# lchdl/DeepWMH

Hardware: NVIDIA B200
Metric: volumes/sec (higher is better)
Workload: dtype f16

## Files before the change

### deepwmh_b200/csrc/conv_tcgen05.cuh

```cuda
#pragma once
#include <cuda.h>
#include <algorithm>
#include <cstdio>
#include <cstdlib>
#include <string>
#include <type_traits>
#include <vector>
#include "common.cuh"
#include "tc_primitives.cuh"

namespace dwmh {

constexpr int TC_WARPS_PER_GROUP = 7;
constexpr int TC_THREADS = 224;
constexpr int TC_TH = 16, TC_TW = 8;
constexpr int TC_PH = 18, TC_PW = 10;
constexpr int TC_PLANE_BYTES = TC_PH * TC_PW * 16;
constexpr int TC_MAX_SA = 4, TC_MAX_NB = 40, TC_MAX_R = 16;
constexpr int TC_SMEM_MAX = 232448;
constexpr int TC_SMEM_RESERVED = 5120;
constexpr int TC_SMEM_RESERVED_FIRST = 10240;
constexpr int TC_FIRST_PITCH = 12;
constexpr int TC_FIRST_SLICE = TC_PH * TC_FIRST_PITCH;
constexpr int TC_FIRST_STAGE_BYTES = 8 * 128 * 16;

struct TcClassDesc { int tapmask, jlo, jcnt, tile0; };

struct TcKParams {
  const void* wpack; void* out; StatPartial* partials;
  int C0, C1, Cout, CB, KC, nkc, nkc0;
  int nclass, Jlo, Jhi, jmax, tiles_per_kc, Din;
  int out32;
  int s222;
  int tconv, CBt, osd, osh, osw, Cout_t;
  TcClassDesc cls[8];
  int D, H, W, tilesH, tilesW, ZB, nzb, ncb;
  int SA, NB, resident, R, fmt;
  const double* xf_sums; const float* xf_gamma; const float* xf_beta; double xf_inv_count; int xform; const void* xf_src;
  const float* fc_src; const SampleMeta* fc_metas; int fc_patch_mode, fc_SY, fc_SZ, first;
  int stagger;
  int G;
  int total_items;
  unsigned long long* prof;
  int dbg;
  uint32_t a_stage_bytes, b_tile_bytes, off_b, off_bar;
};

__global__ void __launch_bounds__(256) stats_reduce_kernel(const StatPartial* __restrict__ partials, double* __restrict__ out,
                                                           int ncb, int CB, int Cout, int ipb, int jn) {
  __shared__ double sh[3][256];
  const int n = blockIdx.x / ncb, cb = blockIdx.x % ncb;
  const int c = threadIdx.x % CB, j = threadIdx.x / CB;
  const StatPartial* base = partials + (size_t)blockIdx.x * ipb * CB + c;
  double cn = 0.0, cm = 0.0, cq = 0.0;
  for (int p = j; p < ipb; p += jn) {
    const float4 v = *reinterpret_cast<const float4*>(base + (size_t)p * CB);
    stat_merge<double>(cn, cm, cq, (double)v.x, (double)v.y, (double)v.z);
  }
  sh[0][threadIdx.x] = cn; sh[1][threadIdx.x] = cm; sh[2][threadIdx.x] = cq;
  __syncthreads();
  if (j == 0) {
    for (int jj = 1; jj < jn; ++jj) stat_merge<double>(cn, cm, cq, sh[0][jj * CB + c], sh[1][jj * CB + c], sh[2][jj * CB + c]);
    double* o = out + ((size_t)n * Cout + (size_t)cb * CB + c) * 2;
    o[0] = cm;
    o[1] = cn > 0.0 ? cq / cn : 0.0;
  }
}

struct RingPos {
  uint32_t idx = 0, phase = 0;
  __device__ __forceinline__ void advance(uint32_t n) { if (++idx == n) { idx = 0; phase ^= 1; } }
  __device__ __forceinline__ RingPos next(uint32_t n) const { RingPos r = *this; r.advance(n); return r; }
};

#define DWMH_TIMED_WAIT(acc, ...) do { if (prof_on) { const long long t__ = clock64(); __VA_ARGS__; acc += clock64() - t__; } else { __VA_ARGS__; } } while (0)

__device__ __forceinline__ uint64_t tc_desc(uint32_t hi, uint32_t lo) { return ((uint64_t)hi << 32) | lo; }

constexpr uint64_t tc_tap_shift_table() {
  uint64_t v = 0;
  for (int sft = 0; sft < 9; ++sft) v |= (uint64_t)((sft / 3) * TC_PW + (sft % 3)) << (5 * sft);
  return v;
}
constexpr uint64_t kTapShift = tc_tap_shift_table();

template <typename T, int KSTEPS, bool SMALL_CB, bool TCONV, bool DUAL, bool XFORM, bool FIRST = false>
__global__ void __launch_bounds__((DUAL ? 2 : 1) * (TC_THREADS + ((FIRST || XFORM) ? 32 : 0)), 1)
conv3_tc_kernel(const __grid_constant__ CUtensorMap tmA0, const __grid_constant__ CUtensorMap tmA1, const TcKParams p) {
  extern __shared__ __align__(1024) uint8_t smem[];
  const uint32_t smem_base = tc::smem_u32(smem);
  const int warp_abs = threadIdx.x >> 5, lane = threadIdx.x & 31;
  constexpr int WPG = TC_WARPS_PER_GROUP;
  constexpr int TPG = WPG * 32;
  constexpr int NG = DUAL ? 2 : 1;
  constexpr bool EXTRA = FIRST || XFORM;
  int g, warp;
  if constexpr (!DUAL) {
    constexpr unsigned char kRole7[7] = {2, 3, 4, 5, 0, 6, 1};
    constexpr unsigned char kRole8[8] = {2, 3, 4, 5, 0, 6, 7, 1};
    g = 0; warp = EXTRA ? kRole8[warp_abs] : kRole7[warp_abs];
  } else if constexpr (!EXTRA) {
    constexpr unsigned char kGroup14[14] = {0, 0, 0, 0, 1, 1, 1, 1, 0, 1, 0, 1, 1, 0};
    constexpr unsigned char kRole14[14] = {2, 3, 4, 5, 2, 3, 4, 5, 0, 0, 6, 6, 1, 1};
    g = kGroup14[warp_abs]; warp = kRole14[warp_abs];
  } else {
    constexpr unsigned char kGroup16[16] = {0, 0, 0, 0, 1, 1, 1, 1, 0, 1, 1, 1, 0, 0, 1, 0};
    constexpr unsigned char kRole16[16] = {2, 3, 4, 5, 2, 3, 4, 5, 0, 0, 6, 7, 6, 7, 1, 1};
    g = kGroup16[warp_abs]; warp = kRole16[warp_abs];
  }
  const bool extra = warp == 7;

  int wi = blockIdx.x * p.G + g;
  const bool idle = wi >= p.total_items;
  if (idle) wi = p.total_items - 1;
  const int tw = wi % p.tilesW; wi /= p.tilesW;
  const int th = wi % p.tilesH; wi /= p.tilesH;
  const int zb = wi % p.nzb; wi /= p.nzb;
  const int cb = wi % p.ncb; wi /= p.ncb;
  const int n = wi;
  const int h0 = th * TC_TH, w0 = tw * TC_TW;
  const int z_lo = zb * p.ZB, z_end = min(p.D, z_lo + p.ZB);
  const uint32_t SA = p.SA, NB = p.NB, R = p.R, CB = p.CB;

  const uint32_t nbar = 3 * SA + 2 * NB + 2 * R;
  const uint32_t bar0 = smem_base + p.off_bar, bar = bar0 + (uint32_t)g * nbar * 8u;
  const uint32_t a_full = bar, a_empty = bar + 8u * SA;
  const uint32_t b_full = bar0 + 16u * SA, b_empty = b_full + 8u * NB;
  const uint32_t acc_full = bar + 16u * SA + 16u * NB, acc_empty = acc_full + 8u * R;
  const uint32_t a_ready = acc_empty + 8u * R;
  const uint32_t a_mma = (XFORM || FIRST) ? a_ready : a_full;
  uint32_t* tmem_ptr_smem = reinterpret_cast<uint32_t*>(smem + p.off_bar + 8 * nbar * p.G);
  const uint32_t aux_off = (p.off_bar + 8u * nbar * (uint32_t)p.G + 16u + 8u) & ~15u;
  float* s_coef = reinterpret_cast<float*>(smem + aux_off) + (size_t)p.G * 2 * CB + (size_t)g * 2 * 64;
  float* s_slice = reinterpret_cast<float*>(smem + aux_off) + (size_t)p.G * 2 * CB + (size_t)p.G * 2 * 64 + (size_t)g * 4 * TC_FIRST_SLICE;
  const uint32_t smem_a = smem_base + (uint32_t)g * SA * p.a_stage_bytes;
  const uint32_t smem_a_d = smem_a & 0x3FFFFu, smem_b_d = (smem_base + p.off_b) & 0x3FFFFu;
  const uint32_t s_full = smem_base + p.off_bar + TC_SMEM_RESERVED_FIRST - 128 + (uint32_t)g * 64u, s_empty = s_full + 32u;

  if (threadIdx.x == 0) {
    if constexpr (!FIRST) {
      tc::prefetch_tensormap(&tmA0);
      tc::prefetch_tensormap(&tmA1);
    }
    for (int gg = 0; gg < p.G; ++gg) {
      const uint32_t bg = bar0 + (uint32_t)gg * nbar * 8u;
      for (uint32_t s_ = 0; s_ < SA; ++s_) { tc::mbar_init(bg + 8 * s_, 1); tc::mbar_init(bg + 8 * (SA + s_), 1); }
      for (uint32_t s_ = 0; s_ < R; ++s_) { tc::mbar_init(bg + 16 * SA + 16 * NB + 8 * s_, 1); tc::mbar_init(bg + 16 * SA + 16 * NB + 8 * (R + s_), 4); }
      for (uint32_t s_ = 0; s_ < SA; ++s_) tc::mbar_init(bg + 16 * SA + 16 * NB + 16 * R + 8 * s_, XFORM ? 3 : 2);
    }
    if constexpr (FIRST)
      for (int gg = 0; gg < p.G; ++gg)
        for (uint32_t s_ = 0; s_ < 4; ++s_) {
          tc::mbar_init(smem_base + p.off_bar + TC_SMEM_RESERVED_FIRST - 128 + gg * 64 + 8 * s_, 1);
          tc::mbar_init(smem_base + p.off_bar + TC_SMEM_RESERVED_FIRST - 128 + gg * 64 + 32 + 8 * s_, 2);
        }
    const uint32_t nactive = (uint32_t)min(p.G, p.total_items - (int)blockIdx.x * p.G);
    for (uint32_t s_ = 0; s_ < NB; ++s_) { tc::mbar_init(b_full + 8 * s_, 1); tc::mbar_init(b_empty + 8 * s_, nactive); }
    tc::fence_barrier_init();
  }
  if (warp_abs == 1) tc::tmem_alloc(tc::smem_u32(tmem_ptr_smem), 512);
  if constexpr (XFORM) {
    for (int i = threadIdx.x; i < p.G * p.C0; i += blockDim.x) {
      const int gg = i / p.C0, c_ = i - gg * p.C0;
      const int item = min((int)blockIdx.x * p.G + gg, p.total_items - 1);
      const int n_gg = item / (p.tilesW * p.tilesH * p.nzb * p.ncb);
      NormParams np{p.xf_sums, p.xf_gamma, p.xf_beta, p.xf_inv_count};
      float a_, b_;
      norm_coeffs(np, n_gg, p.C0, c_, a_, b_);
      float* co = reinterpret_cast<float*>(smem + aux_off) + (size_t)p.G * 2 * CB + (size_t)gg * 2 * 64;
      co[c_] = a_; co[64 + c_] = b_;
    }
  }
  tc::tc_fence_before();
  __syncthreads();
  tc::tc_fence_after();
  const uint32_t tmem = *tmem_ptr_smem + (uint32_t)g * 256u;
  const bool prof_on = (p.dbg & 8) != 0;
  long long w0_ = 0, w1_ = 0, w2_ = 0, w3_ = 0;
  const long long tstart_ = clock64();

  if (idle) {
  } else
  if (FIRST && warp == 7) {
    int ox = 0, oy = 0, oz = 0, flip = 0;
    const float* src = p.fc_src;
    int SY = p.fc_SY, SZ = p.fc_SZ;
    if (p.fc_patch_mode) { src += (size_t)n * p.D * p.H * p.W; SY = p.H; SZ = p.W; }
    else { const SampleMeta m_ = p.fc_metas[n]; ox = m_.ox; oy = m_.oy; oz = m_.oz; flip = m_.flip; }
    int sgoff[6]; bool sin_[6];
#pragma unroll
    for (int i = 0; i < 6; ++i) {
      const int pos = lane + 32 * i;
      const int r = pos / TC_PW, c = pos - r * TC_PW;
// ... 188 lines not shown
            const int c8 = first ? (n * p.nclass + c) * (p.C0 >> 3) + kc * (2 * KSTEPS) : n * (p.C1 >> 3) + (kc - p.nkc0) * (2 * KSTEPS);
            tc::tma_load_4d(smem_a + a.idx * p.a_stage_bytes, first ? &tmA0 : &tmA1, a_full + 8 * a.idx, (w0 - 1) * 8, h0 - 1, t, c8);
          }
          a.advance(SA);
        }
      }
    }
  } else if (warp == 6) {
    const bool leader = tc::elect_one();
    const int ntile = p.nkc * p.tiles_per_kc;
    const uint8_t* wsrc = reinterpret_cast<const uint8_t*>(p.wpack) + (size_t)cb * ntile * p.b_tile_bytes;
    if (p.resident) {
      if (leader && g == 0)
        for (int t = 0; t < ntile; ++t) {
          tc::mbar_arrive_expect_tx(b_full + 8 * t, p.b_tile_bytes);
          tc::bulk_load(smem_base + p.off_b + t * p.b_tile_bytes, wsrc + (size_t)t * p.b_tile_bytes, p.b_tile_bytes, b_full + 8 * t);
        }
    } else if (g == 0) {
      RingPos b;
      for (int t = z_lo - p.Jhi; t <= z_end - 1 - p.Jlo; ++t) {
        if (t < 0 || t >= p.Din) continue;
        for (int c = 0; c < p.nclass; ++c) {
          if (max(t + p.cls[c].jlo, z_lo) > min(t + p.cls[c].jlo + p.cls[c].jcnt - 1, z_end - 1)) continue;
          const int ntaps = __popc(p.cls[c].tapmask);
          for (int kc = 0; kc < p.nkc; ++kc)
            for (int ti = 0; ti < ntaps; ++ti) {
              const int tile = kc * p.tiles_per_kc + p.cls[c].tile0 + ti;
              DWMH_TIMED_WAIT(w0_, tc::mbar_wait(b_empty + 8 * b.idx, b.phase ^ 1, 2));
              if (leader) {
                tc::mbar_arrive_expect_tx(b_full + 8 * b.idx, p.b_tile_bytes);
                tc::bulk_load(smem_base + p.off_b + b.idx * p.b_tile_bytes, wsrc + (size_t)tile * p.b_tile_bytes, p.b_tile_bytes, b_full + 8 * b.idx);
              }
              b.advance(NB);
            }
        }
      }
    }
  } else if (warp == 1) {
    const bool elected = tc::elect_one();
    const bool leader = elected && !(p.dbg & 2);
    if constexpr (FIRST) {
      const uint32_t idesc = tc::instr_desc_f16(p.fmt, 128, (int)CB);
      const uint32_t hi_desc = (128u >> 4) | (1u << 14);
      const uint32_t a_lbo = (2048u >> 4) << 16, b_lbo = ((CB * 16u) >> 4) << 16;
      const uint32_t b_lo0 = (smem_b_d >> 4) | b_lbo;
      tc::mbar_wait(b_full, 0, 5);
      RingPos a, fresh, done;
      for (int t = z_lo; t < z_end; ++t) {
        tc::mbar_wait(acc_empty + 8 * fresh.idx, fresh.phase ^ 1, 3);
        tc::mbar_wait(a_mma + 8 * a.idx, a.phase, 4);
        tc::tc_fence_after();
        if (leader) {
          const uint32_t a_lo0 = ((smem_a_d + a.idx * p.a_stage_bytes) >> 4) | a_lbo;
          const uint32_t col = tmem + fresh.idx * CB;
#pragma unroll
          for (int i = 0; i < 6; ++i) {
            const int achunk = (i == 0 || i == 4) ? 0 : (i == 1 || i == 5) ? 2 : (i == 2 ? 4 : 6);
            tc::umma_f16(col, tc_desc(hi_desc, a_lo0 + achunk * (2048 >> 4)), tc_desc(hi_desc, b_lo0 + i * 2 * CB), idesc, i == 0 ? 0u : 1u);
          }
        }
        if (elected) { tc::umma_commit(a_empty + 8 * a.idx); tc::umma_commit(acc_full + 8 * done.idx); }
        a.advance(SA); fresh.advance(R); done.advance(R);
        __syncwarp();
      }
    } else {
    const uint32_t idesc0 = tc::instr_desc_f16(p.fmt, 128, 0);
    const uint32_t idesc1 = idesc0 | ((CB >> 3) << 17);
    const uint32_t b_lbo16 = (uint32_t)p.jmax * CB;
    const uint32_t kstep_b = 2u * b_lbo16, tile16 = p.b_tile_bytes >> 4;
    const uint32_t a_hi = (uint32_t)((TC_PW * 16) >> 4) | (1u << 14);
    const uint32_t b_hi = (128u >> 4) | (1u << 14);
    const uint32_t a_lbo_field = (uint32_t)(TC_PLANE_BYTES >> 4) << 16;
    const uint32_t b_lo_res = (smem_b_d >> 4) | (b_lbo16 << 16);
    const int t_first = z_lo - p.Jhi, t_last_nominal = z_end - 1 - p.Jlo;
    const int last_t = min(t_last_nominal, p.Din - 1);
    const bool plain = p.nclass == 1 && p.Jlo == -1 && p.Jhi == 1;
    if (p.resident)
      for (int t = 0; t < p.nkc * p.tiles_per_kc; ++t) tc::mbar_wait(b_full + 8 * t, 0, 5);
    if (DUAL && g == 1 && p.stagger > 0) {
      tc::mbar_wait(a_mma, 0, 4);
      const long long t0_ = clock64();
      while (clock64() - t0_ < (long long)p.stagger) { }
    }
    RingPos a, b, fresh, done;
    bool b_peek = false;
    bool a_peek = false;
    uint32_t lo_slot = 0;
    int next_fresh = z_lo, next_done = z_lo, zo_lo_prev = z_lo;
    for (int t = t_first; t <= t_last_nominal; ++t) {
      if (t < 0 || t >= p.Din) continue;
      const int zo_lo = max(t + p.Jlo, z_lo), zo_hi = min(t + p.Jhi, z_end - 1);
      if (zo_lo != zo_lo_prev) { lo_slot = (lo_slot + 1 == R) ? 0 : lo_slot + 1; zo_lo_prev = zo_lo; }
      const int fresh_from = next_fresh;
      while (next_fresh <= zo_hi) {
        DWMH_TIMED_WAIT(w1_, tc::mbar_wait(acc_empty + 8 * fresh.idx, fresh.phase ^ 1, 3));
        fresh.advance(R);
        ++next_fresh;
      }
      if (plain && zo_hi - zo_lo == 2 && R >= 3 && 3 * CB <= 256 && fresh_from == zo_hi) {
        const uint32_t id2 = idesc0 | (((2 * CB) >> 3) << 17), id3 = idesc0 | (((3 * CB) >> 3) << 17);
        auto steady = [&](auto res_c) {
        constexpr bool RES = decltype(res_c)::value;
        for (;;) {
        const uint32_t col = tmem + lo_slot * CB;
        const bool wrap = lo_slot + 3 > R, wrapA = lo_slot + 2 == R;
        const uint32_t idA = wrapA ? id2 : idesc1, idB = wrapA ? idesc1 : id2, offB = wrapA ? 2 * CB : CB;
        const uint32_t col1 = (lo_slot + 1 == R) ? tmem : col + CB, col2 = wrapA ? tmem : tmem + CB;
        for (int kc = 0; kc < p.nkc; ++kc) {
          if (!a_peek) DWMH_TIMED_WAIT(w0_, tc::mbar_wait(a_mma + 8 * a.idx, a.phase, 4));
          tc::tc_fence_after();
          { const RingPos an = a.next(SA); a_peek = tc::mbar_test_wait(a_mma + 8 * an.idx, an.phase); }
          const long long tb_ = prof_on ? clock64() : 0;
          if constexpr (!RES) {
            const uint32_t a_lo0 = ((smem_a_d + a.idx * p.a_stage_bytes) >> 4) | a_lbo_field;
#pragma unroll
            for (int sft = 0; sft < 9; ++sft) {
              if (!b_peek) DWMH_TIMED_WAIT(w1_, tc::mbar_wait(b_full + 8 * b.idx, b.phase, 6));
              tc::tc_fence_after();
              const uint32_t b_lo0 = ((smem_b_d + b.idx * p.b_tile_bytes) >> 4) | (b_lbo16 << 16);
              { const RingPos bn = b.next(NB); b_peek = tc::mbar_test_wait(b_full + 8 * bn.idx, bn.phase); }
              if (leader) {
#pragma unroll
                for (int kk = 0; kk < KSTEPS; ++kk) {
                  const uint64_t adesc = tc_desc(a_hi, a_lo0 + (sft / 3) * TC_PW + (sft % 3) + kk * (2 * TC_PLANE_BYTES >> 4));
                  const uint32_t b0 = b_lo0 + kk * kstep_b;
                  const bool first = sft == 0 && kk == 0 && kc == 0;
                  if (!wrap) {
                    if (first) {
                      tc::umma_f16(col, adesc, tc_desc(b_hi, b0), id2, 1u);
                      tc::umma_f16(col + 2 * CB, adesc, tc_desc(b_hi, b0 + 2 * CB), idesc1, 0u);
                    } else tc::umma_f16(col, adesc, tc_desc(b_hi, b0), id3, 1u);
                  } else if (first) {
                    tc::umma_f16(col, adesc, tc_desc(b_hi, b0), idesc1, 1u);
                    tc::umma_f16(col1, adesc, tc_desc(b_hi, b0 + CB), idesc1, 1u);
                    tc::umma_f16(col2, adesc, tc_desc(b_hi, b0 + 2 * CB), idesc1, 0u);
                  } else {
                    tc::umma_f16(col, adesc, tc_desc(b_hi, b0), idA, 1u);
                    tc::umma_f16(tmem, adesc, tc_desc(b_hi, b0 + offB), idB, 1u);
                  }
                }
              }
              if (elected) tc::umma_commit(b_empty + 8 * b.idx);
              b.advance(NB);
            }
          } else if (leader && !wrap) {
            const uint32_t a_lo0 = ((smem_a_d + a.idx * p.a_stage_bytes) >> 4) | a_lbo_field;
            uint32_t bl = b_lo_res + (uint32_t)kc * 9u * tile16;
#pragma unroll
            for (int sft = 0; sft < 9; ++sft) {
#pragma unroll
              for (int kk = 0; kk < KSTEPS; ++kk) {
                const uint64_t adesc = tc_desc(a_hi, a_lo0 + (sft / 3) * TC_PW + (sft % 3) + kk * (2 * TC_PLANE_BYTES >> 4));
                if (sft == 0 && kk == 0) {
                  if (kc == 0) {
                    tc::umma_f16(col, adesc, tc_desc(b_hi, bl), id2, 1u);
                    tc::umma_f16(col + 2 * CB, adesc, tc_desc(b_hi, bl + 2 * CB), idesc1, 0u);
                  } else tc::umma_f16(col, adesc, tc_desc(b_hi, bl), id3, 1u);
                } else tc::umma_f16(col, adesc, tc_desc(b_hi, bl + kk * kstep_b), id3, 1u);
              }
              bl += tile16;
            }
          } else if (leader) {
            const uint32_t a_lo0 = ((smem_a_d + a.idx * p.a_stage_bytes) >> 4) | a_lbo_field;
            uint32_t bl = b_lo_res + (uint32_t)kc * 9u * tile16;
#pragma unroll
            for (int sft = 0; sft < 9; ++sft) {
#pragma unroll
              for (int kk = 0; kk < KSTEPS; ++kk) {
                const uint64_t adesc = tc_desc(a_hi, a_lo0 + (sft / 3) * TC_PW + (sft % 3) + kk * (2 * TC_PLANE_BYTES >> 4));
// ... 178 lines not shown
            a.advance(SA);
          }
        }
        if (elected) tc::umma_commit(acc_full + 8 * done.idx);
        done.advance(R);
        ++next_done;
        __syncwarp();
        continue;
      }
      const long long tg_ = prof_on ? clock64() : 0;
      bool first_mma = true;
      for (int c = 0; c < p.nclass; ++c) {
        const int dlo = max(t + p.cls[c].jlo, z_lo), dhi = min(t + p.cls[c].jlo + p.cls[c].jcnt - 1, z_end - 1);
        if (dlo > dhi) continue;
        const uint32_t cnt = (uint32_t)(dhi - dlo + 1), r0 = (uint32_t)(dlo - (t + p.cls[c].jlo));
        uint32_t sl = lo_slot + (uint32_t)(dlo - zo_lo);
        if (sl >= R) sl -= R;
        uint32_t nseg = 0, sc0 = 0, sc1 = 0, sc2 = 0, sb0 = 0, sb1 = 0, sb2 = 0, si0 = 0, si1 = 0, si2 = 0;
        {
          uint32_t i = 0;
          while (i < cnt) {
            const uint32_t slot = sl + i < R ? sl + i : sl + i - R;
            uint32_t len = min(cnt - i, R - slot);
            len = min(len, 256u / CB);
            const uint32_t c_ = tmem + slot * CB, b_ = (r0 + i) * CB, d_ = idesc0 | (((len * CB) >> 3) << 17);
            if (nseg == 0) { sc0 = c_; sb0 = b_; si0 = d_; } else if (nseg == 1) { sc1 = c_; sb1 = b_; si1 = d_; } else { sc2 = c_; sb2 = b_; si2 = d_; }
            ++nseg; i += len;
          }
        }
        const int tapmask = p.cls[c].tapmask;
        for (int kc = 0; kc < p.nkc; ++kc) {
          if (!a_peek) DWMH_TIMED_WAIT(w0_, tc::mbar_wait(a_mma + 8 * a.idx, a.phase, 4));
          a_peek = false;
          tc::tc_fence_after();
          const uint32_t a_lo0 = ((smem_a_d + a.idx * p.a_stage_bytes) >> 4) | a_lbo_field;
          uint32_t b_res = b_lo_res + (uint32_t)(kc * p.tiles_per_kc + p.cls[c].tile0) * tile16;
          for (int m = tapmask; m; m &= m - 1) {
            const int sft = __ffs(m) - 1;
            uint32_t b_lo0;
            if (p.resident) { b_lo0 = b_res; b_res += tile16; }
            else {
              if (!b_peek) DWMH_TIMED_WAIT(w1_, tc::mbar_wait(b_full + 8 * b.idx, b.phase, 6));
              tc::tc_fence_after();
              b_lo0 = ((smem_b_d + b.idx * p.b_tile_bytes) >> 4) | (b_lbo16 << 16);
              { const RingPos bn = b.next(NB); b_peek = tc::mbar_test_wait(b_full + 8 * bn.idx, bn.phase); }
            }
            const uint32_t a_lo1 = a_lo0 + (uint32_t)((kTapShift >> (5 * sft)) & 31u);
            if (first_mma) {
              for (uint32_t i = 0; i < cnt; ++i) {
                const uint32_t slot = sl + i < R ? sl + i : sl + i - R;
                if (leader) tc::umma_f16(tmem + slot * CB, tc_desc(a_hi, a_lo1), tc_desc(b_hi, b_lo0 + (r0 + i) * CB), idesc1,
                                         (dlo + (int)i) >= fresh_from ? 0u : 1u);
              }
            }
            if (leader) {
#pragma unroll
              for (int kk = 0; kk < KSTEPS; ++kk) {
                if (kk == 0 && first_mma) continue;
                const uint64_t adesc = tc_desc(a_hi, a_lo1 + kk * (2 * TC_PLANE_BYTES >> 4));
                const uint32_t bl = b_lo0 + kk * kstep_b;
                tc::umma_f16(sc0, adesc, tc_desc(b_hi, bl + sb0), si0, 1u);
                if (nseg > 1) tc::umma_f16(sc1, adesc, tc_desc(b_hi, bl + sb1), si1, 1u);
                if (nseg > 2) tc::umma_f16(sc2, adesc, tc_desc(b_hi, bl + sb2), si2, 1u);
              }
            }
            first_mma = false;
            if (!p.resident) {
              if (elected) tc::umma_commit(b_empty + 8 * b.idx);
              b.advance(NB);
            }
          }
          if (elected) tc::umma_commit(a_empty + 8 * a.idx);
          a.advance(SA);
        }
      }
      const int done_upto = (t == last_t) ? z_end - 1 : t + p.Jlo;
      while (next_done <= done_upto) {
        if (elected) tc::umma_commit(acc_full + 8 * done.idx);
        done.advance(R);
        ++next_done;
      }
      __syncwarp();
      if (prof_on) w3_ += clock64() - tg_;
    }
    }
  } else {
    const int q = warp_abs & 3;
    const int row = q * 32 + lane;
    const int h = h0 + (row >> 3), w = w0 + (row & 7);
    const bool valid = h < p.H && w < p.W && !(p.dbg & 4);
    const uint32_t tm_lane = tmem + ((uint32_t)(q * 32) << 16);
    const int nch = CB >> 4;
    if constexpr (TCONV) {
      const int Ho = p.H * p.osh, Wo = p.W * p.osw;
      const size_t Vo = (size_t)p.D * p.osd * Ho * Wo;
      uint4* out_n = reinterpret_cast<uint4*>(p.out) + (size_t)n * (p.Cout_t >> 3) * Vo;
      uint32_t slot = 0, phase = 0;
      for (int t = z_lo; t < z_end; ++t) {
        DWMH_TIMED_WAIT(w0_, tc::mbar_wait(acc_full + 8 * slot, phase, 7));
        tc::tc_fence_after();
        if (p.osw == 2) {
          const int cpp = p.CBt >> 4;
          int chq = 0;
          for (int qa = 0; qa < p.osd; ++qa)
            for (int qb = 0; qb < p.osh; ++qb, chq += 2 * cpp)
              for (int cc = 0; cc < cpp; ++cc) {
                uint32_t r[2][16];
                tc::tmem_ld16(tm_lane + slot * CB + (chq + cc) * 16, r[0]);
                tc::tmem_ld16(tm_lane + slot * CB + (chq + cpp + cc) * 16, r[1]);
                tc::tmem_ld_wait();
                if (valid) {
                  float a0[16], a1[16];
#pragma unroll
                  for (int i = 0; i < 16; ++i) { a0[i] = __uint_as_float(r[0][i]); a1[i] = __uint_as_float(r[1][i]); }
                  uint4* o = out_n + (size_t)((cb * p.CBt + cc * 16) >> 3) * Vo + ((size_t)(t * p.osd + qa) * Ho + (h * p.osh + qb)) * Wo + (size_t)w * 2;
                  st_global_256(o, pack8<T>(a0), pack8<T>(a1));
                  st_global_256(o + Vo, pack8<T>(a0 + 8), pack8<T>(a1 + 8));
                }
              }
        } else {
        int cofs = 0, qa = 0, qb = 0, qw = 0;
        for (int ch = 0; ch < nch; ch += 2) {
          uint32_t r[2][16];
          tc::tmem_ld16(tm_lane + slot * CB + ch * 16, r[0]);
          tc::tmem_ld16(tm_lane + slot * CB + ch * 16 + 16, r[1]);
          tc::tmem_ld_wait();
#pragma unroll
          for (int u = 0; u < 2; ++u) {
            float a[16];
#pragma unroll
            for (int i = 0; i < 16; ++i) a[i] = __uint_as_float(r[u][i]);
            if (valid) {
              uint4* o = out_n + (size_t)((cb * p.CBt + cofs) >> 3) * Vo + ((size_t)(t * p.osd + qa) * Ho + (h * p.osh + qb)) * Wo + (w * p.osw + qw);
              o[0] = pack8<T>(a);
              o[Vo] = pack8<T>(a + 8);
            }
            cofs += 16;
            if (cofs == p.CBt) {
              cofs = 0;
              if (++qw == p.osw) { qw = 0; if (++qb == p.osh) { qb = 0; ++qa; } }
            }
          }
        }
        }
        tc::tc_fence_before();
        __syncwarp();
        if (lane == 0) tc::mbar_arrive(acc_empty + 8 * slot);
        if (++slot == R) { slot = 0; phase ^= 1; }
      }
    } else {
    constexpr int NACC = SMALL_CB ? 32 : 8;
    float rs[NACC], rq[NACC];
#pragma unroll
    for (int i = 0; i < NACC; ++i) { rs[i] = 0.f; rq[i] = 0.f; }
    float cnt = 0.f;
    const float nvw = (float)__popc(__ballot_sync(0xffffffffu, valid));
    const size_t V = (size_t)p.D * p.H * p.W;
    uint4* out_base = reinterpret_cast<uint4*>(p.out) + ((size_t)n * (p.Cout >> 3) + (size_t)cb * (CB >> 3)) * V;
    uint32_t slot = 0, phase = 0;
    for (int zo = z_lo; zo < z_end; ++zo) {
      DWMH_TIMED_WAIT(w0_, tc::mbar_wait(acc_full + 8 * slot, phase, 7));
      tc::tc_fence_after();
      uint4* outp = out_base + ((size_t)zo * p.H + h) * p.W + w;
      float wgt_new, cnt_prev = cnt;
      if constexpr (SMALL_CB) { cnt += 1.f; wgt_new = __frcp_rn(cnt); }
      else { cnt += nvw; wgt_new = nvw > 0.f ? __fdividef(nvw, cnt) : 0.f; }
#pragma unroll
      for (int ch = 0; ch < (SMALL_CB ? 2 : 8); ++ch) {
        if (ch < nch) {
          uint32_t r[16];
          tc::tmem_ld16(tm_lane + slot * CB + ch * 16, r);
          tc::tmem_ld_wait();
          float a[16];
#pragma unroll
          for (int i = 0; i < 16; ++i) a[i] = __uint_as_float(r[i]);
          if (valid) {
            if (p.out32) {
              float4* o32 = reinterpret_cast<float4*>(p.out) + 2 * (size_t)(outp - reinterpret_cast<uint4*>(p.out));
              o32[(size_t)(2 * ch) * V * 2] = make_float4(a[0], a[1], a[2], a[3]);
              o32[(size_t)(2 * ch) * V * 2 + 1] = make_float4(a[4], a[5], a[6], a[7]);
              o32[(size_t)(2 * ch + 1) * V * 2] = make_float4(a[8], a[9], a[10], a[11]);
              o32[(size_t)(2 * ch + 1) * V * 2 + 1] = make_float4(a[12], a[13], a[14], a[15]);
            } else {
              outp[(size_t)(2 * ch) * V] = pack8<T>(a);
              outp[(size_t)(2 * ch + 1) * V] = pack8<T>(a + 8);
            }
          }
          if constexpr (SMALL_CB) {
            if (valid) {
#pragma unroll
              for (int i = 0; i < 16; ++i) {
                const float d = a[i] - rs[ch * 16 + i];
                rs[ch * 16 + i] = fmaf(d, wgt_new, rs[ch * 16 + i]);
                rq[ch * 16 + i] = fmaf(d, a[i] - rs[ch * 16 + i], rq[ch * 16 + i]);
              }
            }
          } else {
            float b[16];
#pragma unroll
            for (int i = 0; i < 16; ++i) {
              const float piv = __shfl_sync(0xffffffffu, rs[ch], i);
              a[i] = valid ? a[i] - piv : 0.f;
              b[i] = a[i] * a[i];
            }
#pragma unroll
            for (int k = 8; k >= 1; k >>= 1) {
              const bool up = (lane & k) != 0;
#pragma unroll
              for (int i = 0; i < k; ++i) {
                const float sa_ = up ? a[i] : a[i + k], ka_ = up ? a[i + k] : a[i];
                const float sb_ = up ? b[i] : b[i + k], kb_ = up ? b[i + k] : b[i];
                a[i] = ka_ + __shfl_xor_sync(0xffffffffu, sa_, k);
                b[i] = kb_ + __shfl_xor_sync(0xffffffffu, sb_, k);
              }
            }
            const float S = a[0] + __shfl_xor_sync(0xffffffffu, a[0], 16), Q = b[0] + __shfl_xor_sync(0xffffffffu, b[0], 16);
            if (nvw > 0.f) {
              const float dm = S / nvw;
              rq[ch] += fmaf(-S, dm, Q) + dm * dm * cnt_prev * wgt_new;
              rs[ch] = fmaf(dm, wgt_new, rs[ch]);
            }
          }
        }
      }
      tc::tc_fence_before();
      __syncwarp();
      if (lane == 0) tc::mbar_arrive(acc_empty + 8 * slot);
      if (++slot == R) { slot = 0; phase ^= 1; }
    }
    StatPartial* pout = reinterpret_cast<StatPartial*>(smem + (size_t)g * SA * p.a_stage_bytes) + (size_t)q * CB;
    if constexpr (SMALL_CB) {
      const float n_row = valid ? cnt : 0.f;
#pragma unroll
      for (int ch = 0; ch < 2; ++ch) {
        if (ch < nch) {
          float a[16], b[16];
#pragma unroll
          for (int i = 0; i < 16; ++i) { a[i] = rs[ch * 16 + i]; b[i] = rq[ch * 16 + i]; }
          float nn = n_row;
#pragma unroll
          for (int k = 8; k >= 1; k >>= 1) {
            const bool up = (lane & k) != 0;
            const float np_ = __shfl_xor_sync(0xffffffffu, nn, k);
            const float nt = nn + np_, wp = nt > 0.f ? np_ / nt : 0.f;
#pragma unroll
            for (int i = 0; i < k; ++i) {
              const float sa_ = up ? a[i] : a[i + k], ka_ = up ? a[i + k] : a[i];
              const float sb_ = up ? b[i] : b[i + k], kb_ = up ? b[i + k] : b[i];
              const float pm = __shfl_xor_sync(0xffffffffu, sa_, k), pq = __shfl_xor_sync(0xffffffffu, sb_, k);
              const float d = pm - ka_;
              a[i] = fmaf(d, wp, ka_);
              b[i] = kb_ + pq + d * d * nn * wp;
            }
            nn = nt;
          }
          const float np_ = __shfl_xor_sync(0xffffffffu, nn, 16), pm = __shfl_xor_sync(0xffffffffu, a[0], 16), pq = __shfl_xor_sync(0xffffffffu, b[0], 16);
          float m_ = a[0], q_ = b[0];
          stat_merge<float>(nn, m_, q_, np_, pm, pq);
          if (lane < 16) *reinterpret_cast<float4*>(pout + ch * 16 + lane) = make_float4(nn, m_, q_, 0.f);
        }
      }
    } else if (lane < 16) {
#pragma unroll
      for (int ch = 0; ch < 8; ++ch)
        if (ch < nch) *reinterpret_cast<float4*>(pout + ch * 16 + lane) = make_float4(cnt, rs[ch], rq[ch], 0.f);
    }
    }
  }
  if (prof_on && lane == 0 && g == 0 && (warp <= 2 || warp == 6)) {
    const int role = warp == 6 ? 3 : warp;
    atomicAdd(p.prof + role * 4 + 0, (unsigned long long)w0_);
    atomicAdd(p.prof + role * 4 + 1, (unsigned long long)w1_);
    atomicAdd(p.prof + role * 4 + 2, (unsigned long long)(clock64() - tstart_));
    atomicAdd(p.prof + role * 4 + 3, (unsigned long long)w2_);
    if (role == 1) atomicAdd(p.prof + 3, (unsigned long long)w3_);
  }
  tc::tc_fence_before();
  __syncthreads();
  if constexpr (!TCONV) {
    for (int i = threadIdx.x; i < p.G * (int)CB; i += blockDim.x) {
      const int gg = i / (int)CB, c_ = i - gg * (int)CB;
      if ((int)blockIdx.x * p.G + gg >= p.total_items) continue;
      const StatPartial* pin = reinterpret_cast<const StatPartial*>(smem + (size_t)gg * SA * p.a_stage_bytes) + c_;
      float4 v = *reinterpret_cast<const float4*>(pin);
#pragma unroll
      for (int qq = 1; qq < 4; ++qq) {
        const float4 u = *reinterpret_cast<const float4*>(pin + (size_t)qq * CB);
        stat_merge<float>(v.x, v.y, v.z, u.x, u.y, u.z);
      }
      *reinterpret_cast<float4*>(p.partials + (size_t)(blockIdx.x * p.G + gg) * CB + c_) = v;
    }
  }
  if (warp_abs == 1) tc::tmem_dealloc(tmem, 512);
}

struct TcLayer {
  bool enabled = false;
  int ms0[6] = {0, 0, 0, 0, 0, 0}, ms1[6] = {0, 0, 0, 0, 0, 0};
  bool map_bf16 = false;
  bool xform_ok = false;
  CUtensorMap tm0, tm1;
  void* wpack = nullptr;
  TcKParams kp{};
  size_t smem_bytes = 0;
};

inline void tc_free(TcLayer& t) {
  if (t.wpack) cudaFree(t.wpack);
  t.wpack = nullptr;
  t.enabled = false;
}
// ... 86 lines not shown
        else { cd_.jlo = 0; cd_.jcnt = 2; cls_kd[c] = {2, 0}; }
        for (int dy = 0; dy < 3; ++dy)
          for (int dx = 0; dx < 3; ++dx) {
            int kh = -1, kw = -1;
            if (sh == 1) kh = dy; else if (ph == 0) { if (dy == 1) kh = 1; } else { if (dy == 0) kh = 0; else if (dy == 1) kh = 2; }
            if (sw == 1) kw = dx; else if (pw == 0) { if (dx == 1) kw = 1; } else { if (dx == 0) kw = 0; else if (dx == 1) kw = 2; }
            if (kh < 0 || kw < 0) continue;
            cd_.tapmask |= 1 << (dy * 3 + dx);
            cls_taps[c].push_back({kh, kw});
          }
        tile0 += (int)cls_taps[c].size();
      }
  kp.tiles_per_kc = tile0;
  kp.s222 = (sd == 2 && sh == 2 && sw == 2 && kp.nclass == 8 && tile0 == 18) ? 1 : 0;
  for (int c = 0; c < 8 && kp.s222; ++c) {
    const int cd = c >> 2, ph = (c >> 1) & 1, pw = c & 1;
    int mask = 0;
    for (int iy = 0; iy < (ph ? 2 : 1); ++iy)
      for (int ix = 0; ix < (pw ? 2 : 1); ++ix) mask |= 1 << ((ph ? iy : 1) * 3 + (pw ? ix : 1));
    const TcClassDesc& d = kp.cls[c];
    if (d.tapmask != mask || d.tile0 != cd * 9 + (ph ? (pw ? 5 : 3) : (pw ? 1 : 0)) || d.jlo != 0 || d.jcnt != (cd == 0 ? 2 : 1)) kp.s222 = 0;
  }
  int KC0 = 64;
  while (KC0 > 16 && (c0 % KC0 || c1 % KC0)) KC0 >>= 1;
  const int budget = TC_SMEM_MAX - TC_SMEM_RESERVED;
  int KC = 0, CB = 0, SA = 0, NB = 0, resident = 0, G = 1;
  static int allow_dual = -1;
  if (allow_dual < 0) { const char* e = getenv("DWMH_TC_DUAL"); allow_dual = e ? atoi(e) : 1; }
  for (int kc = KC0; kc >= 16 && !CB && allow_dual; kc >>= 1) {
    const int a_stage = kc * 360, ntile = (cin / kc) * kp.tiles_per_kc;
    if (ntile > TC_MAX_NB) continue;
    for (int cbt = std::min(cout, 64); cbt >= 32; cbt -= 16) {
      if (cout % cbt) continue;
      const long long btot = (long long)ntile * kp.jmax * cbt * kc * 2;
      if (btot + 2LL * 3 * a_stage <= budget) {
        KC = kc; CB = cbt; resident = 1; NB = ntile; G = 2;
        SA = (int)std::min<long long>(tc_max_sa(), (budget - btot) / (2LL * a_stage));
        break;
      }
    }
  }
  for (int kc = KC0; kc >= 32 && !CB && allow_dual; kc >>= 1) {
    const int a_stage = kc * 360;
    for (int cbt = std::min(cout, 64); cbt >= 32; cbt -= 16) {
      if (cout % cbt) continue;
      if (256 / cbt < kp.jmax + 1) continue;
      const int b_tile = kp.jmax * cbt * kc * 2;
      const int nb = (budget - 2 * 3 * a_stage) / b_tile;
      if (nb >= 3) { KC = kc; CB = cbt; resident = 0; SA = 3; NB = std::min(nb, TC_MAX_NB); G = 2; break; }
    }
  }
  for (int kc = KC0; kc >= 16 && !CB; kc >>= 1) {
    const int a_stage = kc * 360, ntile = (cin / kc) * kp.tiles_per_kc;
    if (ntile <= TC_MAX_NB) {
      for (int cbt = std::min(cout, 128); cbt >= 16; cbt -= 16) {
        if (cout % cbt) continue;
        if (cbt < 32 && cbt != cout) break;
        const long long btot = (long long)ntile * kp.jmax * cbt * kc * 2;
        if (btot + 2LL * a_stage <= budget) {
          KC = kc; CB = cbt; resident = 1; NB = ntile;
          SA = (int)std::min<long long>(tc_max_sa(), (budget - btot) / a_stage);
          break;
        }
      }
    }
    if (!CB) {
      for (int cbt = std::min(cout, 128); cbt >= 16; cbt -= 16) {
        if (cout % cbt) continue;
        const int b_tile = kp.jmax * cbt * kc * 2;
        const int nb = (budget - 3 * a_stage) / b_tile;
        if (nb >= 3) { KC = kc; CB = cbt; resident = 0; SA = 3; NB = std::min(nb, TC_MAX_NB); break; }
      }
    }
  }
  if (!CB) return 0;
  kp.C0 = c0; kp.C1 = c1; kp.Cout = cout; kp.CB = CB; kp.KC = KC; kp.nkc = cin / KC; kp.nkc0 = c0 / KC;
  kp.D = out_sp[0]; kp.H = out_sp[1]; kp.W = out_sp[2];
  kp.tilesH = (kp.H + TC_TH - 1) / TC_TH; kp.tilesW = (kp.W + TC_TW - 1) / TC_TW;
  kp.ncb = cout / CB; kp.SA = SA; kp.NB = NB; kp.resident = resident; kp.G = G;
  kp.xf_src = nullptr;
  kp.xform = 0; kp.xf_sums = nullptr; kp.xf_gamma = nullptr; kp.xf_beta = nullptr; kp.xf_inv_count = 0.0;
  t.xform_ok = !strided && kd == 3 && resident && c1 == 0 && KC == 32 && (cin == 32 || cin == 64) && CB <= 32 && SA >= 3;
  kp.R = std::min(TC_MAX_R, (512 / G) / CB);
  kp.fmt = bf16 ? 1 : 0;
  kp.a_stage_bytes = KC * 360; kp.b_tile_bytes = kp.jmax * CB * KC * 2;
  kp.off_b = G * SA * kp.a_stage_bytes;
  kp.off_bar = kp.off_b + NB * kp.b_tile_bytes;
  kp.off_bar = (kp.off_bar + 127) & ~127u;
  t.smem_bytes = kp.off_bar + TC_SMEM_RESERVED;
  if (t.smem_bytes > TC_SMEM_MAX) { *why = "internal: shared memory plan exceeds 227 KB"; return 1; }
  if (t.smem_bytes < 120 * 1024) t.smem_bytes = 120 * 1024;
  kp.out = out;
  const size_t tile_elems = (size_t)(KC / 8) * kp.jmax * CB * 8;
  const int ntile = kp.nkc * kp.tiles_per_kc;
  std::vector<uint16_t> pk((size_t)kp.ncb * ntile * tile_elems, 0);
  for (int cb = 0; cb < kp.ncb; ++cb)
    for (int kc = 0; kc < kp.nkc; ++kc)
      for (int c = 0; c < kp.nclass; ++c)
        for (size_t ti = 0; ti < cls_taps[c].size(); ++ti) {
          uint16_t* tile = pk.data() + ((size_t)cb * ntile + (size_t)kc * kp.tiles_per_kc + kp.cls[c].tile0 + ti) * tile_elems;
          for (int k8 = 0; k8 < KC / 8; ++k8)
            for (int r = 0; r < kp.cls[c].jcnt; ++r)
              for (int co_ = 0; co_ < CB; ++co_)
                for (int e = 0; e < 8; ++e) {
                  const int co = cb * CB + co_, ci = kc * KC + k8 * 8 + e;
                  const float v = w[((size_t)co * cin + ci) * (kd * 9) + cls_kd[c][r] * 9 + cls_taps[c][ti].kh * 3 + cls_taps[c][ti].kw];
                  tile[((size_t)k8 * kp.jmax * CB + (size_t)r * CB + co_) * 8 + e] = tc_to_bits(v, bf16);
                }
        }
  if (cudaMalloc(&t.wpack, pk.size() * 2) != cudaSuccess) { *why = "cudaMalloc(wpack) failed"; return 1; }
  if (cudaMemcpy(t.wpack, pk.data(), pk.size() * 2, cudaMemcpyHostToDevice) != cudaSuccess) { *why = "cudaMemcpy(wpack) failed"; return 1; }
  kp.wpack = t.wpack;
  t.map_bf16 = bf16;
  { const int a0[6] = {maxN * kp.nclass, c0, in_sp[0] / sd, in_sp[1] / sh, in_sp[2] / sw, KC}; for (int i = 0; i < 6; ++i) t.ms0[i] = a0[i]; }
  { const int a1[6] = {c1 > 0 ? maxN : 0, c1, in_sp[0], in_sp[1], in_sp[2], KC}; for (int i = 0; i < 6; ++i) t.ms1[i] = a1[i]; }
  if (tc_remap(t, in0, in1, why)) return 1;
  t.enabled = true;
  return 0;
}

inline int tc_prepare_tconv(TcLayer& t, const std::vector<float>& w, int cin, int cout, const int s[3], const int in_sp[3],
                            int maxN, bool bf16, const void* in0, void* out, std::string* why) {
  t.enabled = false;
  why->clear();
  if (cin % 16 || cout % 16) return 0;
  const int nco = s[0] * s[1] * s[2];
  int CBt = 256 / nco;
  while (CBt >= 16 && (cout % CBt || CBt % 16)) CBt -= 16;
  if (CBt < 16) return 0;
  TcKParams& kp = t.kp;
  kp = TcKParams{};
  kp.tconv = 1; kp.CBt = CBt; kp.osd = s[0]; kp.osh = s[1]; kp.osw = s[2]; kp.Cout_t = cout;
  kp.nclass = 1; kp.Jlo = 0; kp.Jhi = 0; kp.jmax = 1; kp.tiles_per_kc = 1; kp.Din = in_sp[0];
  kp.cls[0] = TcClassDesc{1 << 4, 0, 1, 0};
  const int CB = nco * CBt;
  if (CB % 32) return 0;
  int KC = 64;
  while (KC > 16 && cin % KC) KC >>= 1;
  const int budget = TC_SMEM_MAX - TC_SMEM_RESERVED;
  const int a_stage = KC * 360, b_tile = CB * KC * 2, nkc = cin / KC;
  int SA, NB, resident;
  if (nkc <= TC_MAX_NB && (long long)nkc * b_tile + 2LL * a_stage <= budget) {
    resident = 1; NB = nkc; SA = (int)std::min<long long>(TC_MAX_SA, (budget - (long long)nkc * b_tile) / a_stage);
  } else {
    resident = 0; SA = 3; NB = std::min((budget - 3 * a_stage) / b_tile, TC_MAX_NB);
    if (NB < 2) return 0;
  }
  kp.C0 = cin; kp.C1 = 0; kp.Cout = CB * (cout / CBt); kp.CB = CB; kp.KC = KC; kp.nkc = nkc; kp.nkc0 = nkc;
  kp.D = in_sp[0]; kp.H = in_sp[1]; kp.W = in_sp[2];
  kp.tilesH = (kp.H + TC_TH - 1) / TC_TH; kp.tilesW = (kp.W + TC_TW - 1) / TC_TW;
  kp.ncb = cout / CBt; kp.SA = SA; kp.NB = NB; kp.resident = resident;
  kp.R = 512 / CB; kp.fmt = bf16 ? 1 : 0; kp.G = 1;
  kp.a_stage_bytes = a_stage; kp.b_tile_bytes = b_tile;
  kp.off_b = SA * a_stage;
  kp.off_bar = (kp.off_b + NB * b_tile + 127) & ~127u;
  t.smem_bytes = kp.off_bar + TC_SMEM_RESERVED;
  if (t.smem_bytes > TC_SMEM_MAX) { *why = "internal: shared memory plan exceeds 227 KB"; return 1; }
  if (t.smem_bytes < 120 * 1024) t.smem_bytes = 120 * 1024;
  kp.out = out;
  const int taps = nco;
  const size_t tile_elems = (size_t)(KC / 8) * CB * 8;
  std::vector<uint16_t> pk((size_t)kp.ncb * nkc * tile_elems, 0);
  for (int cb = 0; cb < kp.ncb; ++cb)
    for (int kc = 0; kc < nkc; ++kc) {
      uint16_t* tile = pk.data() + ((size_t)cb * nkc + kc) * tile_elems;
      for (int k8 = 0; k8 < KC / 8; ++k8)
// ... 182 lines not shown
```

### deepwmh_b200/csrc/tc_primitives.cuh

```cuda
#pragma once
#include <cuda.h>
#include <cuda_runtime.h>
#include <stdint.h>

namespace dwmh {
namespace tc {

__device__ __forceinline__ uint32_t smem_u32(const void* p) { return (uint32_t)__cvta_generic_to_shared(p); }

__device__ __forceinline__ void mbar_init(uint32_t bar, uint32_t count) {
  asm volatile("mbarrier.init.shared::cta.b64 [%0], %1;" ::"r"(bar), "r"(count));
}
__device__ __forceinline__ void fence_barrier_init() { asm volatile("fence.mbarrier_init.release.cluster;" ::: "memory"); }
__device__ __forceinline__ void mbar_arrive(uint32_t bar) {
  asm volatile("mbarrier.arrive.shared::cta.b64 _, [%0];" ::"r"(bar) : "memory");
}
__device__ __forceinline__ void mbar_arrive_expect_tx(uint32_t bar, uint32_t bytes) {
  asm volatile("mbarrier.arrive.expect_tx.shared::cta.b64 _, [%0], %1;" ::"r"(bar), "r"(bytes) : "memory");
}
__device__ __forceinline__ bool mbar_try_wait(uint32_t bar, uint32_t parity) {
  uint32_t ok;
  asm volatile("{\n .reg .pred p;\n mbarrier.try_wait.parity.shared::cta.b64 p, [%1], %2;\n selp.u32 %0, 1, 0, p;\n}"
               : "=r"(ok) : "r"(bar), "r"(parity) : "memory");
  return ok != 0;
}
__device__ __forceinline__ bool mbar_test_wait(uint32_t bar, uint32_t parity) {
  uint32_t ok;
  asm volatile("{\n .reg .pred p;\n mbarrier.test_wait.parity.shared::cta.b64 p, [%1], %2;\n selp.u32 %0, 1, 0, p;\n}"
               : "=r"(ok) : "r"(bar), "r"(parity) : "memory");
  return ok != 0;
}
__device__ __forceinline__ void mbar_wait(uint32_t bar, uint32_t parity, int tag) {
  uint32_t spins = 0;
  while (!mbar_try_wait(bar, parity)) {
    if (++spins > (1u << 26)) { printf("dwmh tc: mbarrier timeout tag=%d block=%d thread=%d\n", tag, blockIdx.x, threadIdx.x); __trap(); }
  }
}
__device__ __forceinline__ bool elect_one() {
  uint32_t pred;
  asm volatile("{\n .reg .pred P;\n elect.sync _|P, 0xffffffff;\n selp.u32 %0, 1, 0, P;\n}" : "=r"(pred));
  return pred != 0;
}
__device__ __forceinline__ void fence_proxy_async() { asm volatile("fence.proxy.async.shared::cta;" ::: "memory"); }

__device__ __forceinline__ void prefetch_tensormap(const CUtensorMap* m) {
  asm volatile("prefetch.tensormap [%0];" ::"l"(reinterpret_cast<uint64_t>(m)) : "memory");
}
__device__ __forceinline__ void tma_load_4d(uint32_t dst, const CUtensorMap* m, uint32_t bar, int c0, int c1, int c2, int c3) {
  asm volatile("cp.async.bulk.tensor.4d.shared::cluster.global.tile.mbarrier::complete_tx::bytes [%0], [%1, {%3, %4, %5, %6}], [%2];"
               ::"r"(dst), "l"(reinterpret_cast<uint64_t>(m)), "r"(bar), "r"(c0), "r"(c1), "r"(c2), "r"(c3) : "memory");
}
__device__ __forceinline__ void tma_load_5d(uint32_t dst, const CUtensorMap* m, uint32_t bar, int c0, int c1, int c2, int c3, int c4) {
  asm volatile("cp.async.bulk.tensor.5d.shared::cluster.global.tile.mbarrier::complete_tx::bytes [%0], [%1, {%3, %4, %5, %6, %7}], [%2];"
               ::"r"(dst), "l"(reinterpret_cast<uint64_t>(m)), "r"(bar), "r"(c0), "r"(c1), "r"(c2), "r"(c3), "r"(c4) : "memory");
}
__device__ __forceinline__ void bulk_load(uint32_t dst, const void* src, uint32_t bytes, uint32_t bar) {
  asm volatile("cp.async.bulk.shared::cluster.global.mbarrier::complete_tx::bytes [%0], [%1], %2, [%3];"
               ::"r"(dst), "l"(reinterpret_cast<uint64_t>(src)), "r"(bytes), "r"(bar) : "memory");
}

__device__ __forceinline__ void tmem_alloc(uint32_t smem_dst, uint32_t ncols) {
  asm volatile("tcgen05.alloc.cta_group::1.sync.aligned.shared::cta.b32 [%0], %1;" ::"r"(smem_dst), "r"(ncols) : "memory");
  asm volatile("tcgen05.relinquish_alloc_permit.cta_group::1.sync.aligned;" ::: "memory");
}
__device__ __forceinline__ void tmem_dealloc(uint32_t taddr, uint32_t ncols) {
  asm volatile("tcgen05.dealloc.cta_group::1.sync.aligned.b32 %0, %1;" ::"r"(taddr), "r"(ncols) : "memory");
}
__device__ __forceinline__ void tc_fence_before() { asm volatile("tcgen05.fence::before_thread_sync;" ::: "memory"); }
__device__ __forceinline__ void tc_fence_after() { asm volatile("tcgen05.fence::after_thread_sync;" ::: "memory"); }

__device__ __forceinline__ void umma_f16(uint32_t d_tmem, uint64_t adesc, uint64_t bdesc, uint32_t idesc, uint32_t accumulate) {
  asm volatile("{\n .reg .pred p;\n setp.ne.b32 p, %4, 0;\n tcgen05.mma.cta_group::1.kind::f16 [%0], %1, %2, %3, p;\n}"
               ::"r"(d_tmem), "l"(adesc), "l"(bdesc), "r"(idesc), "r"(accumulate) : "memory");
}
__device__ __forceinline__ void umma_commit(uint32_t bar) {
  asm volatile("tcgen05.commit.cta_group::1.mbarrier::arrive::one.shared::cluster.b64 [%0];" ::"r"(bar) : "memory");
}

__device__ __forceinline__ void tmem_ld16(uint32_t taddr, uint32_t r[16]) {
  asm volatile("tcgen05.ld.sync.aligned.32x32b.x16.b32 {%0,%1,%2,%3,%4,%5,%6,%7,%8,%9,%10,%11,%12,%13,%14,%15}, [%16];"
               : "=r"(r[0]), "=r"(r[1]), "=r"(r[2]), "=r"(r[3]), "=r"(r[4]), "=r"(r[5]), "=r"(r[6]), "=r"(r[7]),
                 "=r"(r[8]), "=r"(r[9]), "=r"(r[10]), "=r"(r[11]), "=r"(r[12]), "=r"(r[13]), "=r"(r[14]), "=r"(r[15])
               : "r"(taddr) : "memory");
}
__device__ __forceinline__ void tmem_ld_wait() { asm volatile("tcgen05.wait::ld.sync.aligned;" ::: "memory"); }
__device__ __forceinline__ void tmem_st16_zero(uint32_t taddr) {
  const uint32_t z = 0;
  asm volatile("tcgen05.st.sync.aligned.32x32b.x16.b32 [%0], {%1,%1,%1,%1,%1,%1,%1,%1,%1,%1,%1,%1,%1,%1,%1,%1};" ::"r"(taddr), "r"(z) : "memory");
}
__device__ __forceinline__ void tmem_st_wait() { asm volatile("tcgen05.wait::st.sync.aligned;" ::: "memory"); }

__device__ __forceinline__ uint64_t smem_desc_kmajor_noswizzle(uint32_t addr, uint32_t lbo_bytes, uint32_t sbo_bytes) {
  uint64_t d = 0;
  d |= (uint64_t)((addr >> 4) & 0x3FFF);
  d |= (uint64_t)((lbo_bytes >> 4) & 0x3FFF) << 16;
  d |= (uint64_t)((sbo_bytes >> 4) & 0x3FFF) << 32;
  d |= (uint64_t)1 << 46;
  return d;
}
__host__ __device__ __forceinline__ uint32_t instr_desc_f16(int fmt , int M, int N) {
  return (1u << 4) | ((uint32_t)fmt << 7) | ((uint32_t)fmt << 10) | ((uint32_t)(N >> 3) << 17) | ((uint32_t)(M >> 4) << 24);
}

}
}
```

Measured before the change: 8.295.

## Add restart ring accumulation scheme for plain 3-tap depth conv in TMEM

Adds a new MMA schedule for the plain kd=3 small-CB case. Each input depth plane is multiplied once against all three depth taps with a single N=3*CB MMA into a rotating ring of TMEM slots. The epilogue sums the two overlapping slots at wrap boundaries and zeroes slots before releasing them. This replaces the class/fresh/done bookkeeping and is meant to cut MMA issue count and accumulate-flag logic. In exchange it adds extra TMEM loads in the epilogue, zeroing stores, and more complex slot synchronisation.

```diff
diff --git a/deepwmh_b200/csrc/conv_tcgen05.cuh b/deepwmh_b200/csrc/conv_tcgen05.cuh
--- a/deepwmh_b200/csrc/conv_tcgen05.cuh
+++ b/deepwmh_b200/csrc/conv_tcgen05.cuh
@@ -36,6 +36,7 @@
   TcClassDesc cls[8];
   int D, H, W, tilesH, tilesW, ZB, nzb, ncb;
   int SA, NB, resident, R, fmt;
+  int restart;
   const double* xf_sums; const float* xf_gamma; const float* xf_beta; double xf_inv_count; int xform; const void* xf_src;
   const float* fc_src; const SampleMeta* fc_metas; int fc_patch_mode, fc_SY, fc_SZ, first;
   int stagger;
@@ -71,6 +72,14 @@
   uint32_t idx = 0, phase = 0;
   __device__ __forceinline__ void advance(uint32_t n) { if (++idx == n) { idx = 0; phase ^= 1; } }
   __device__ __forceinline__ RingPos next(uint32_t n) const { RingPos r = *this; r.advance(n); return r; }
+};
+
+struct TcPlaneSlots {
+  uint32_t last = 0, phase = 0, shift = 0;
+  __device__ __forceinline__ uint32_t first() const { return last < 2 ? last + shift : last; }
+  __device__ __forceinline__ void advance(uint32_t span, uint32_t shift_after) {
+    if (++last == span) { last = 0; phase ^= 1; shift = shift_after; }
+  }
 };
 
 #define DWMH_TIMED_WAIT(acc, ...) do { if (prof_on) { const long long t__ = clock64(); __VA_ARGS__; acc += clock64() - t__; } else { __VA_ARGS__; } } while (0)
@@ -109,6 +118,8 @@
     g = kGroup16[warp_abs]; warp = kRole16[warp_abs];
   }
   const bool extra = warp == 7;
+  constexpr bool RING_OK = SMALL_CB && !TCONV && !FIRST;
+  const bool restart = RING_OK && p.restart != 0;
 
   int wi = blockIdx.x * p.G + g;
   const bool idle = wi >= p.total_items;
@@ -463,9 +474,69 @@
       const long long t0_ = clock64();
       while (clock64() - t0_ < (long long)p.stagger) { }
     }
-    RingPos a, b, fresh, done;
+    RingPos a, b;
     bool b_peek = false;
     bool a_peek = false;
+    if (restart) {
+      const uint32_t id3 = idesc0 | (((3 * CB) >> 3) << 17);
+      const int nwin = z_end - z_lo + 2;
+      auto run = [&](auto res_c) {
+        constexpr bool RES = decltype(res_c)::value;
+        TcPlaneSlots ps;
+        for (int i = 0; i < nwin; ++i, ps.advance(R - 2, R - 2)) {
+          const int t = z_lo - 1 + i;
+          const uint32_t lo = ps.last;
+          for (uint32_t s_ = lo == 0 ? 0 : lo + 2; s_ <= lo + 2; ++s_)
+            DWMH_TIMED_WAIT(w1_, tc::mbar_wait(acc_empty + 8 * s_, ps.phase, 3));
+          if (t >= 0 && t < p.Din) {
+            const uint32_t col = tmem + lo * CB;
+            for (int kc = 0; kc < p.nkc; ++kc) {
+              if (!a_peek) DWMH_TIMED_WAIT(w0_, tc::mbar_wait(a_mma + 8 * a.idx, a.phase, 4));
+              tc::tc_fence_after();
+              { const RingPos an = a.next(SA); a_peek = tc::mbar_test_wait(a_mma + 8 * an.idx, an.phase); }
+              const long long tb_ = prof_on ? clock64() : 0;
+              const uint32_t a_lo0 = ((smem_a_d + a.idx * p.a_stage_bytes) >> 4) | a_lbo_field;
+              if constexpr (!RES) {
+#pragma unroll
+                for (int sft = 0; sft < 9; ++sft) {
+                  if (!b_peek) DWMH_TIMED_WAIT(w1_, tc::mbar_wait(b_full + 8 * b.idx, b.phase, 6));
+                  tc::tc_fence_after();
+                  const uint32_t b_lo0 = ((smem_b_d + b.idx * p.b_tile_bytes) >> 4) | (b_lbo16 << 16);
+                  { const RingPos bn = b.next(NB); b_peek = tc::mbar_test_wait(b_full + 8 * bn.idx, bn.phase); }
+                  if (leader) {
+#pragma unroll
+                    for (int kk = 0; kk < KSTEPS; ++kk) {
+                      const uint64_t adesc = tc_desc(a_hi, a_lo0 + (sft / 3) * TC_PW + (sft % 3) + kk * (2 * TC_PLANE_BYTES >> 4));
+                      tc::umma_f16(col, adesc, tc_desc(b_hi, b_lo0 + kk * kstep_b), id3, 1u);
+                    }
+                  }
+                  if (elected) tc::umma_commit(b_empty + 8 * b.idx);
+                  b.advance(NB);
+                }
+              } else if (leader) {
+                uint32_t bl = b_lo_res + (uint32_t)kc * 9u * tile16;
+#pragma unroll
+                for (int sft = 0; sft < 9; ++sft) {
+#pragma unroll
+                  for (int kk = 0; kk < KSTEPS; ++kk) {
+                    const uint64_t adesc = tc_desc(a_hi, a_lo0 + (sft / 3) * TC_PW + (sft % 3) + kk * (2 * TC_PLANE_BYTES >> 4));
+                    tc::umma_f16(col, adesc, tc_desc(b_hi, bl + kk * kstep_b), id3, 1u);
+                  }
+                  bl += tile16;
+                }
+              }
+              if (prof_on) w2_ += clock64() - tb_;
+              if (elected) tc::umma_commit(a_empty + 8 * a.idx);
+              a.advance(SA);
+            }
+          }
+          if (elected) tc::umma_commit(acc_full + 8 * lo);
+          __syncwarp();
+        }
+      };
+      if (p.resident) run(std::true_type{}); else run(std::false_type{});
+    } else {
+    RingPos fresh, done;
     uint32_t lo_slot = 0;
     int next_fresh = z_lo, next_done = z_lo, zo_lo_prev = z_lo;
     for (int t = t_first; t <= t_last_nominal; ++t) {
@@ -810,6 +881,7 @@
       }
       __syncwarp();
       if (prof_on) w3_ += clock64() - tg_;
+    }
     }
     }
   } else {
@@ -885,10 +957,29 @@
     const float nvw = (float)__popc(__ballot_sync(0xffffffffu, valid));
     const size_t V = (size_t)p.D * p.H * p.W;
     uint4* out_base = reinterpret_cast<uint4*>(p.out) + ((size_t)n * (p.Cout >> 3) + (size_t)cb * (CB >> 3)) * V;
-    uint32_t slot = 0, phase = 0;
-    for (int zo = z_lo; zo < z_end; ++zo) {
-      DWMH_TIMED_WAIT(w0_, tc::mbar_wait(acc_full + 8 * slot, phase, 7));
+    auto release = [&](uint32_t s_first, uint32_t s_last) {
+      if (restart) {
+        for (int ch = 0; ch < nch; ++ch) {
+          tc::tmem_st16_zero(tm_lane + s_last * CB + ch * 16);
+          if (s_first != s_last) tc::tmem_st16_zero(tm_lane + s_first * CB + ch * 16);
+        }
+        tc::tmem_st_wait();
+      }
+      tc::tc_fence_before();
+      __syncwarp();
+      if (lane == 0) {
+        tc::mbar_arrive(acc_empty + 8 * s_last);
+        if (s_first != s_last) tc::mbar_arrive(acc_empty + 8 * s_first);
+      }
+    };
+    if (restart)
+      for (uint32_t s_ = 0; s_ < R; ++s_) release(s_, s_);
+    TcPlaneSlots ps;
+    for (int zo = restart ? z_lo - 2 : z_lo; zo < z_end; ++zo, ps.advance(restart ? R - 2 : R, restart ? R - 2 : 0)) {
+      const uint32_t slot = ps.last, first = restart ? ps.first() : slot;
+      DWMH_TIMED_WAIT(w0_, tc::mbar_wait(acc_full + 8 * slot, ps.phase, 7));
       tc::tc_fence_after();
+      if (zo < z_lo) { release(first, slot); continue; }
       uint4* outp = out_base + ((size_t)zo * p.H + h) * p.W + w;
       float wgt_new, cnt_prev = cnt;
       if constexpr (SMALL_CB) { cnt += 1.f; wgt_new = __frcp_rn(cnt); }
@@ -902,6 +993,16 @@
           float a[16];
 #pragma unroll
           for (int i = 0; i < 16; ++i) a[i] = __uint_as_float(r[i]);
+          if (first != slot) {
+#pragma unroll
+            for (int hf = 0; hf < 16; hf += 8) {
+              uint32_t r8[8];
+              tc::tmem_ld8(tm_lane + first * CB + ch * 16 + hf, r8);
+              tc::tmem_ld_wait();
+#pragma unroll
+              for (int i = 0; i < 8; ++i) a[hf + i] = __uint_as_float(r8[i]) + a[hf + i];
+            }
+          }
           if (valid) {
             if (p.out32) {
               float4* o32 = reinterpret_cast<float4*>(p.out) + 2 * (size_t)(outp - reinterpret_cast<uint4*>(p.out));
@@ -951,10 +1052,7 @@
           }
         }
       }
-      tc::tc_fence_before();
-      __syncwarp();
-      if (lane == 0) tc::mbar_arrive(acc_empty + 8 * slot);
-      if (++slot == R) { slot = 0; phase ^= 1; }
+      release(first, slot);
     }
     StatPartial* pout = reinterpret_cast<StatPartial*>(smem + (size_t)g * SA * p.a_stage_bytes) + (size_t)q * CB;
     if constexpr (SMALL_CB) {
@@ -1207,6 +1305,7 @@
   kp.xform = 0; kp.xf_sums = nullptr; kp.xf_gamma = nullptr; kp.xf_beta = nullptr; kp.xf_inv_count = 0.0;
   t.xform_ok = !strided && kd == 3 && resident && c1 == 0 && KC == 32 && (cin == 32 || cin == 64) && CB <= 32 && SA >= 3;
   kp.R = std::min(TC_MAX_R, (512 / G) / CB);
+  kp.restart = (kp.nclass == 1 && kp.Jlo == -1 && kp.Jhi == 1 && kp.R >= 6 && CB <= 32) ? 1 : 0;
   kp.fmt = bf16 ? 1 : 0;
   kp.a_stage_bytes = KC * 360; kp.b_tile_bytes = kp.jmax * CB * KC * 2;
   kp.off_b = G * SA * kp.a_stage_bytes;
diff --git a/deepwmh_b200/csrc/tc_primitives.cuh b/deepwmh_b200/csrc/tc_primitives.cuh
--- a/deepwmh_b200/csrc/tc_primitives.cuh
+++ b/deepwmh_b200/csrc/tc_primitives.cuh
@@ -83,6 +83,10 @@
                  "=r"(r[8]), "=r"(r[9]), "=r"(r[10]), "=r"(r[11]), "=r"(r[12]), "=r"(r[13]), "=r"(r[14]), "=r"(r[15])
                : "r"(taddr) : "memory");
 }
+__device__ __forceinline__ void tmem_ld8(uint32_t taddr, uint32_t r[8]) {
+  asm volatile("tcgen05.ld.sync.aligned.32x32b.x8.b32 {%0,%1,%2,%3,%4,%5,%6,%7}, [%8];"
+               : "=r"(r[0]), "=r"(r[1]), "=r"(r[2]), "=r"(r[3]), "=r"(r[4]), "=r"(r[5]), "=r"(r[6]), "=r"(r[7]) : "r"(taddr) : "memory");
+}
 __device__ __forceinline__ void tmem_ld_wait() { asm volatile("tcgen05.wait::ld.sync.aligned;" ::: "memory"); }
 __device__ __forceinline__ void tmem_st16_zero(uint32_t taddr) {
   const uint32_t z = 0;
```

Result: no change. 8.368 (median of 6 runs) (+0.9%).
